# florianwechsung/alfi

Measured on AMD Instinct MI355X. Metric: V-cycles/sec on ldc3d P2-P0 (DoF*smooths/sec in dof_smooths_per_s), higher is better.
Workload: dtype f64

## Files before the change

### alfi_amd/csrc/api_patches.hip

```cpp
#include <optional>
#include "api_internal.h"
#include "find_groups.h"

static_assert(PLAN_E_ARG == ALFI_E_ARG, "the planners (patch_plan.h) return the C ABI's code");


static void free_f32(alfi_level* L) {
  if (L->inv32 && --L->ctx->f32_levels == 0) {
    dev_free(L->ctx->f32_work);
    L->ctx->f32_work = nullptr;
    L->ctx->f32_work_doubles = 0;
  }
  dev_free(L->inv32);
  dev_free(L->inv32_ptr);
  L->inv32 = nullptr;
  L->inv32_ptr = nullptr;
  L->inv32_floats = 0;
  std::vector<int64_t>().swap(L->f32_ptr);
  if (L->held == HELD_F32) set_held(L, HELD_NONE);
}

static int inv_to_placeholder(alfi_level* L) {
  dev_free(L->inv);
  L->inv = nullptr;
// ... 512 lines not shown
  std::vector<std::vector<int32_t>> si(ng);
  for (int g = 0; g < ng; ++g) {
    mat[g].resize((size_t)cond_group_doubles(g_m[g], g_sc[g]));
    si[g].resize(g_sc[g]);
    ALFI_HIP_CHECK(ctx, down(mat[g].data(), cd.mat + g_mat[g], sizeof(double) * mat[g].size()));
    ALFI_HIP_CHECK(ctx, down(si[g].data(), cd.sidx + g_sidx[g], sizeof(int32_t) * g_sc[g]));
  }
  std::vector<double> x(n), y(n), rhs(s);
  for (int j = 0; j < n; ++j) {
    std::fill(x.begin(), x.end(), 0.0);
    x[j] = 1.0;
    for (int i = 0; i < s; ++i) rhs[i] = x[nI + i];
    for (int g = 0; g < ng; ++g) {
      const int m = g_m[g], sc = g_sc[g], o = g_off[g], ldm = cond_ldim(m), ldsc = cond_ldim(sc);
      const double* X = mat[g].data();
      const double* B = X + (size_t)ldm * m;
      for (int i = 0; i < m; ++i) {
        double acc = 0.0;
        for (int k = 0; k < m; ++k) acc += X[(size_t)k * ldm + i] * x[o + k];
        y[o + i] = acc;
      }
      for (int i = 0; i < sc; ++i) {
        double acc = 0.0;
        for (int k = 0; k < m; ++k) acc += B[(size_t)k * ldsc + i] * y[o + k];
        rhs[si[g][i]] -= acc;
      }
    }
    for (int i = 0; i < s; ++i) {
      double acc = 0.0;
      for (int k = 0; k < s; ++k) acc += sinv[patch_inv_index(i, k, s, ld)] * rhs[k];
      y[nI + i] = acc;
    }
    for (int g = 0; g < ng; ++g) {
      const int m = g_m[g], sc = g_sc[g], o = g_off[g], ldm = cond_ldim(m);
      const double* W = mat[g].data() + (size_t)ldm * m + (size_t)cond_ldim(sc) * m;
      for (int i = 0; i < m; ++i) {
        double acc = 0.0;
        for (int k = 0; k < sc; ++k) acc += W[(size_t)k * ldm + i] * y[nI + si[g][k]];
        y[o + i] -= acc;
// ... 31 lines not shown
```

### alfi_amd/csrc/cond_layout.h

```cpp
#pragma once
#include <cstdint>

#ifdef __HIPCC__
#define ALFI_HD __host__ __device__
#else
#define ALFI_HD
#endif

struct CondChunk {
  int64_t off;
  int64_t ubase;
  int64_t sidx0;
  int64_t stage_off;
  int32_t xq0, xq1;
  int32_t bq0, bq1;
  int32_t e0, ne;
  int32_t u0, nu;
  int32_t nI;
  int32_t xp0, bp0;
  int32_t pad;
};

#ifndef ALFI_COND_SIGMA_ROWS
#define ALFI_COND_SIGMA_ROWS 64
#endif
constexpr int COND_SIGMA_ROWS = ALFI_COND_SIGMA_ROWS;

constexpr int64_t COND_PER_PATCH_MIN = 1024;

ALFI_HD inline int cond_patch_waves(int max_pairs) {
#ifdef ALFI_COND_WAVES_FORCE
  (void)max_pairs;
  return ALFI_COND_WAVES_FORCE;
#else
  return max_pairs <= 64 ? 1 : max_pairs <= 128 ? 2 : max_pairs <= 256 ? 4 : 8;
#endif
}

ALFI_HD inline int cond_ldim(int rows) { return (rows + 1) & ~1; }
ALFI_HD inline int cond_pairs(int rows) { return (rows + 1) / 2; }
ALFI_HD inline int64_t cond_group_doubles(int m, int sc) {
  return (int64_t)cond_ldim(m) * m + (int64_t)cond_ldim(sc) * m + (int64_t)cond_ldim(m) * sc;
}
```

### alfi_amd/csrc/kernels_bigpatch.hip

```cpp
#include <algorithm>
#include <cstdlib>
#include <vector>
#include "common.h"
#include "row_piece.h"
#include "cond_apply.h"

constexpr int BIG_NB = 64;
constexpr int BIG_MAX_NP = PATCH_MAX;

template <int BS>
__global__ __launch_bounds__(256) void big_gather_kernel(int64_t p0, const int32_t* __restrict__ rowptr,
                                                          const int32_t* __restrict__ colidx,
                                                          const double* __restrict__ vals, int flat,
                                                          const int64_t* __restrict__ patch_ptr,
                                                          const int32_t* __restrict__ patch_dofs,
                                                          const int64_t* __restrict__ scr_ptr, double* __restrict__ scr) {
  __shared__ int32_t dofs_s[BIG_MAX_NP];
  const int64_t p = p0 + blockIdx.y;
  const int64_t off = patch_ptr[p];
  const int n = (int)(patch_ptr[p + 1] - off);
  const int N = (n + BIG_NB - 1) / BIG_NB * BIG_NB;
  double* S = scr + scr_ptr[blockIdx.y];
  for (int i = threadIdx.x; i < n; i += 256) dofs_s[i] = patch_dofs[off + i];
  const int chunk = (N + gridDim.x - 1) / gridDim.x;
// ... 749 lines not shown
    const int m = cd.g_m[g], sc = cd.g_sc[g];
    const int ldm = cond_ldim(m), ldsc = cond_ldim(sc);
    const double* B = cd.mat + cd.g_mat[g] + (int64_t)ldm * m;
    const double* W = B + (int64_t)ldsc * m;
    const int32_t* si = cd.sidx + cd.g_sidx[g];
    for (int e = threadIdx.x; e < sc * sc; e += 256) {
      const int i = e % sc, j = e / sc;
      double acc = 0.0;
      for (int k = 0; k < m; ++k) acc = __builtin_fma(B[(int64_t)k * ldsc + i], W[(int64_t)j * ldm + k], acc);
      S[(int64_t)si[i] * N + si[j]] -= acc;
    }
    __syncthreads();
  }
}



template <bool NT, int COND_WAVES, int RU>
__global__ __launch_bounds__(64 * COND_WAVES) void cond_front_kernel(int64_t p0, int64_t p1, CondDev cd,
                                                                     const int64_t* __restrict__ patch_ptr,
                                                                     const int64_t* __restrict__ stage_ptr,
                                                                     const double* __restrict__ x, double* __restrict__ stage,
                                                                     int ordered) {
  extern __shared__ double cond_dsmem[];
  constexpr int NT_ = 64 * COND_WAVES;
  if (p0 + blockIdx.x >= p1) return;
  const int64_t p = ordered ? cd.order[blockIdx.x] : p0 + blockIdx.x;
  const int64_t off = patch_ptr[p];
  const int n = (int)(patch_ptr[p + 1] - off);
  const int nI = cd.p_nI[p];
  const int s = n - nI;
  const int64_t uo0 = cd.uptr[p];
  double* xs = cond_dsmem;
  double* ts = xs + n;
  double* us = ts + nI;
  for (int i0 = threadIdx.x; i0 < n; i0 += 4 * NT_) {
    int32_t d[4];
#pragma unroll
    for (int u = 0; u < 4; ++u) d[u] = (i0 + u * NT_ < n) ? cd.dofs[off + i0 + u * NT_] : 0;
    double v[4];
#pragma unroll
    for (int u = 0; u < 4; ++u) v[u] = (i0 + u * NT_ < n) ? x[d[u]] : 0.0;
#pragma unroll
    for (int u = 0; u < 4; ++u)
      if (i0 + u * NT_ < n) xs[i0 + u * NT_] = v[u];
  }
  __syncthreads();
  double* tmp = cd.tmp + off;
  const int64_t xp0 = cd.xp_ptr[p], bp0 = cd.bp_ptr[p];
  const int nxp = (int)(cd.xp_ptr[p + 1] - xp0), nbp = (int)(cd.bp_ptr[p + 1] - bp0);
  for (int q0 = 0; q0 < nxp; q0 += NT_) {
    const int q = q0 + threadIdx.x;
    const bool act = q < nxp;
    const int32_t g = act ? cd.xp_grp[xp0 + q] : (int32_t)cd.gptr[p];
    const int m = cd.g_m[g], o = cd.g_off[g], i = 2 * (q - cd.g_xp[g]);
    double t0 = 0.0, t1 = 0.0;
    cond_row2_dot<NT, RU>(cd.mat + cd.g_mat[g] + i, cond_ldim(m), act ? m : 0, xs + o, t0, t1);
    if (act) {
      ts[o + i] = t0;
      tmp[o + i] = t0;
      if (i + 1 < m) {
        ts[o + i + 1] = t1;
        tmp[o + i + 1] = t1;
      }
    }
  }
  __syncthreads();
  for (int q0 = 0; q0 < nbp; q0 += NT_) {
    const int q = q0 + threadIdx.x;
    const bool act = q < nbp;
    const int32_t g = act ? cd.bp_grp[bp0 + q] : (int32_t)cd.gptr[p];
    const int m = cd.g_m[g], sc = cd.g_sc[g], j = 2 * (q - cd.g_bp[g]);
    const int64_t ue = uo0 + cd.g_uoff[g] + j;
    const int32_t d0 = act ? cd.u_dst[ue] : 0, d1 = (act && j + 1 < sc) ? cd.u_dst[ue + 1] : 0;
    double u0 = 0.0, u1 = 0.0;
    cond_row2_dot<NT, RU>(cd.mat + cd.g_mat[g] + (int64_t)cond_ldim(m) * m + j, cond_ldim(sc), act ? m : 0,
                          ts + cd.g_off[g], u0, u1);
    if (act) {
      us[d0] = u0;
      if (j + 1 < sc) us[d1] = u1;
    }
  }
  __syncthreads();
  const int64_t srow0 = cd.sptr[p];
  const int32_t qb = cd.s_uptr[srow0];
  double* rhs = stage + stage_ptr[p] + nI;
  for (int i = threadIdx.x; i < s; i += NT_) {
    double acc = xs[nI + i];
    const int32_t qe = cd.s_uptr[srow0 + i + 1] - qb;
    for (int32_t q = cd.s_uptr[srow0 + i] - qb; q < qe; ++q) acc -= us[q];
    rhs[i] = acc;
  }
}

template <bool NT>
// ... 19 lines not shown
  const int lg = __builtin_ctz(R) - 1;
  const bool ahead = a < b && s <= BIG_U * (64 >> lg);
  big_d2 sv[BIG_U];
  if (ahead) big_block_prefetch<NT>(cd.sinv + cd.sinv_ptr[p] + (int64_t)row0 * s + (a - row0), P, s, lg, lane, sv);
  for (int i = threadIdx.x; i < s; i += 256) cond_dsmem[i] = rhs[i];
  __syncthreads();
  double* ys = cd.tmp + off + nI;
  if (ahead) {
    big_block_finish(sv, s, lg, cond_dsmem, lane, ys + a, s - a);
    if (a + R < b) big_rows<NT>(cd.sinv + cd.sinv_ptr[p], s, ld, a + R, b, cond_dsmem, lane, ys);
  } else if (a < b) {
    big_rows<NT>(cd.sinv + cd.sinv_ptr[p], s, ld, a, b, cond_dsmem, lane, ys);
  }
}

template <bool NT, int COND_WAVES, int RU>
__global__ __launch_bounds__(64 * COND_WAVES) void cond_back_kernel(int64_t p0, int64_t p1, CondDev cd,
                                                                    const int64_t* __restrict__ patch_ptr,
                                                                    const int64_t* __restrict__ stage_ptr,
                                                                    double* __restrict__ stage, int ordered) {
  extern __shared__ double cond_dsmem[];
  constexpr int NT_ = 64 * COND_WAVES;
  if (p0 + blockIdx.x >= p1) return;
  const int64_t p = ordered ? cd.order[blockIdx.x] : p0 + blockIdx.x;
  const int64_t off = patch_ptr[p];
  const int n = (int)(patch_ptr[p + 1] - off);
  const int nI = cd.p_nI[p];
  const int s = n - nI;
  const int uo = (int)(cd.uptr[p + 1] - cd.uptr[p]);
  const int64_t g0 = cd.gptr[p];
  double* ys = cond_dsmem;
  double* yg = ys + s;
  const double* tmp = cd.tmp + off;
  for (int i = threadIdx.x; i < s; i += NT_) ys[i] = tmp[nI + i];
  const int32_t* si = cd.sidx + (uo > 0 ? cd.g_sidx[g0] : 0);
  int32_t sq[4];
#pragma unroll
  for (int u = 0; u < 4; ++u) sq[u] = (threadIdx.x + u * NT_ < uo) ? si[threadIdx.x + u * NT_] : 0;
  __syncthreads();
#pragma unroll
  for (int u = 0; u < 4; ++u)
    if (threadIdx.x + u * NT_ < uo) yg[threadIdx.x + u * NT_] = ys[sq[u]];
  for (int q = threadIdx.x + 4 * NT_; q < uo; q += NT_) yg[q] = ys[si[q]];
  __syncthreads();
  double* out = stage + stage_ptr[p];
  const int64_t xp0 = cd.xp_ptr[p];
  const int nxp = (int)(cd.xp_ptr[p + 1] - xp0);
  for (int q0 = 0; q0 < nxp; q0 += NT_) {
// ... 66 lines not shown
  d.boff = cd.g_mat[g] + (int64_t)cond_ldim(m) * m + j;
  d.ld = cond_ldim(sc);
  d.m = m;
  d.o = cd.g_off[g];
  d.d0 = cd.u_dst[ue];
  d.d1 = j + 1 < sc ? cd.u_dst[ue + 1] : -1;
  d.pad = 0;
  return d;
}

template <bool NT>
__global__ __launch_bounds__(256) void cond_gfront_kernel(int64_t k0, CondDev cd, const double* __restrict__ x) {
  extern __shared__ double cond_dsmem[];
  const CondChunk c = cd.gc[k0 + blockIdx.x];
  double* xs = cond_dsmem;
  double* ts = xs + c.ne;
  const int tid = threadIdx.x;
  const bool xact = c.xq0 + tid < c.xq1, bact = c.bq0 + tid < c.bq1;
  const CondXPair xd = cond_xpair(cd, c, c.xq0 + tid, xact);
  const CondBPair bd = cond_bpair(cd, c, c.bq0 + tid, bact);
  for (int i = tid; i < c.ne; i += 256) xs[i] = x[cd.dofs[c.off + c.e0 + i]];
  big_d2 xa[COND_U], ba[COND_U];
  cond_row2_prefetch<NT>(cd.mat + xd.xoff, xd.ld, xact ? xd.m : 0, xa);
  cond_row2_prefetch<NT>(cd.mat + bd.boff, bd.ld, bact ? bd.m : 0, ba);
  __syncthreads();
  double* tmp = cd.tmp + c.off;
  {
    double t0 = 0.0, t1 = 0.0;
    cond_row2_finish<NT>(cd.mat + xd.xoff, xd.ld, xact ? xd.m : 0, xs + (xd.o - c.e0), xa, t0, t1);
    if (xact) {
      const int e = xd.o + xd.i;
      ts[e - c.e0] = t0;
      tmp[e] = t0;
      if (xd.sl1 >= 0) {
        ts[e - c.e0 + 1] = t1;
        tmp[e + 1] = t1;
      }
    }
  }
  __syncthreads();
  {
    double v0 = 0.0, v1 = 0.0;
    cond_row2_finish<NT>(cd.mat + bd.boff, bd.ld, bact ? bd.m : 0, ts + (bd.o - c.e0), ba, v0, v1);
    if (bact) {
      cd.ubuf[c.ubase + bd.d0] = v0;
      if (bd.d1 >= 0) cd.ubuf[c.ubase + bd.d1] = v1;
    }
  }
}

template <bool NT>
__global__ __launch_bounds__(256) void cond_gsigma_kernel(int64_t c0, CondDev cd, const int64_t* __restrict__ patch_ptr,
                                                          const int64_t* __restrict__ stage_ptr, const double* __restrict__ x,
                                                          double* __restrict__ stage) {
  extern __shared__ double cond_dsmem[];
  const int64_t c = c0 + blockIdx.x;
  const int64_t p = cd.ch_patch[c];
  const int r0 = cd.ch_row[c];
// ... 106 lines not shown
        hipLaunchKernelGGL(cond_fill_kernel<3>, dim3((unsigned)nb), block, lds, ctx->stream, p0, K->cd, K->patch_ptr,
                           K->patch_dofs, K->A.rowptr, K->A.colidx, K->A.vals, K->A.flat, d_scr_ptr, dst, K->status);
      const int64_t ga = K->cplan.gptr[p0], gb = K->cplan.gptr[p0 + nb];
      if (gb > ga && pivot_groups) {
        const size_t glds = (size_t)(COND_GMAX * COND_GMAX + 64 * COND_GMAX) * sizeof(double) + COND_GMAX * sizeof(int);
        (void)hipFuncSetAttribute(reinterpret_cast<const void*>(&cond_group_pivot_kernel),
                                  hipFuncAttributeMaxDynamicSharedMemorySize, (int)glds);
        hipLaunchKernelGGL(cond_group_pivot_kernel, dim3((unsigned)(gb - ga)), dim3(64), glds, ctx->stream, ga, K->cd, K->status);
      } else if (gb > ga && K->cplan.max_m <= 16)
        hipLaunchKernelGGL(cond_group16_kernel, dim3((unsigned)((gb - ga + 15) / 16)), block, 0, ctx->stream, ga, gb, K->cd,
                           K->status);
      else if (gb > ga)
        hipLaunchKernelGGL(cond_group_kernel, dim3((unsigned)((gb - ga + 3) / 4)), block, 0, ctx->stream, ga, gb, K->cd,
                           K->status);
      hipLaunchKernelGGL(cond_schur_kernel, dim3((unsigned)nb), block, 0, ctx->stream, p0, K->cd, K->patch_ptr, d_scr_ptr, dst);
    } else if (C) {
      const int64_t n = C->n, N = (n + BIG_NB - 1) / BIG_NB * BIG_NB;
      hipLaunchKernelGGL(coarse_pad_kernel, dim3(8192), block, 0, ctx->stream, n, N, dst);
      if (C->bs == 2)
        hipLaunchKernelGGL(coarse_scatter_kernel<2>, dim3(4096), block, 0, ctx->stream, C->A.nbrows, C->A.rowptr, C->A.colidx,
                           C->A.vals, C->A.flat, N, dst);
      else
        hipLaunchKernelGGL(coarse_scatter_kernel<3>, dim3(4096), block, 0, ctx->stream, C->A.nbrows, C->A.rowptr, C->A.colidx,
                           C->A.vals, C->A.flat, N, dst);
    } else if (T) {
      hipLaunchKernelGGL(big_dense_fill_kernel, dim3(64, (unsigned)nb), block, 0, ctx->stream, p0, T->m, T->KII, T->DII,
                         T->nu, T->gamma, d_scr_ptr, dst);
    } else {
      if (L->bs == 2)
        hipLaunchKernelGGL(big_gather_kernel<2>, dim3(16, (unsigned)nb), block, 0, ctx->stream, p0, L->A.rowptr, L->A.colidx,
// ... 206 lines not shown
    const int64_t k0 = L->cplan.gcptr[p0], k1 = L->cplan.gcptr[p1];
    const size_t lds_f = (size_t)L->cplan.lds_gfront, lds_b = (size_t)L->cplan.lds_gback;
    const size_t lds_s = (size_t)(L->cplan.max_s + 2 + COND_SIGMA_ROWS) * sizeof(double);
    if (k1 > k0)
      hipLaunchKernelGGL((cond_gfront_kernel<false>), dim3((unsigned)(k1 - k0)), dim3(256), lds_f, ctx->stream, k0, L->cd, x);
    if (c1 > c0)
      hipLaunchKernelGGL((cond_gsigma_kernel<true>), dim3((unsigned)(c1 - c0)), dim3(256), lds_s, ctx->stream, c0, L->cd,
                         L->patch_ptr, L->stage_ptr, x, L->stage);
    if (k1 > k0)
      hipLaunchKernelGGL((cond_gback_kernel<false>), dim3((unsigned)(k1 - k0)), dim3(256), lds_b, ctx->stream, k0, L->cd,
                         L->stage);
    ALFI_HIP_CHECK(ctx, hipGetLastError());
    return 0;
  }
  const size_t lds_f = (size_t)L->cplan.lds_front, lds_s = (size_t)(L->cplan.max_s + 2) * sizeof(double);
  const size_t lds_b = (size_t)L->cplan.lds_back;
#define ALFI_COND_LAUNCH3(WV)                                                                                             \
  do {                                                                                                                    \
    if (lds_f > 64 * 1024)                                                                                                \
      ALFI_HIP_CHECK(ctx, hipFuncSetAttribute(reinterpret_cast<const void*>(&cond_front_kernel<false, WV, 8>),            \
                                              hipFuncAttributeMaxDynamicSharedMemorySize, (int)lds_f));                   \
    hipLaunchKernelGGL((cond_front_kernel<false, WV, 8>), dim3(grid.x), dim3(64 * WV), lds_f, ctx->stream, p0, p1, L->cd, \
                       L->patch_ptr, L->stage_ptr, x, L->stage, ordered);                                                 \
    if (c1 > c0)                                                                                                          \
      hipLaunchKernelGGL((cond_sigma_kernel<true>), dim3((unsigned)(c1 - c0)), dim3(256), lds_s, ctx->stream, c0, L->cd,  \
                         L->patch_ptr, L->stage_ptr, L->stage);                                                           \
    if (lds_b > 64 * 1024)                                                                                                \
      ALFI_HIP_CHECK(ctx, hipFuncSetAttribute(reinterpret_cast<const void*>(&cond_back_kernel<false, WV, 8>),             \
                                              hipFuncAttributeMaxDynamicSharedMemorySize, (int)lds_b));                   \
    hipLaunchKernelGGL((cond_back_kernel<false, WV, 8>), dim3(grid.x), dim3(64 * WV), lds_b, ctx->stream, p0, p1, L->cd,  \
                       L->patch_ptr, L->stage_ptr, L->stage, ordered);                                                    \
  } while (0)
#ifdef ALFI_COND_WAVES_FORCE
  ALFI_COND_LAUNCH3(ALFI_COND_WAVES_FORCE);
#else
  switch (cond_patch_waves(L->cplan.max_pairs)) {
    case 1: ALFI_COND_LAUNCH3(1); break;
    case 2: ALFI_COND_LAUNCH3(2); break;
    case 4: ALFI_COND_LAUNCH3(4); break;
    default: ALFI_COND_LAUNCH3(8); break;
  }
#endif
#undef ALFI_COND_LAUNCH3
  ALFI_HIP_CHECK(ctx, hipGetLastError());
  return 0;
}

#include "mf_coarse.h"
```

### alfi_amd/csrc/kernels_block_cond.hip

```cpp
#include "common.h"
#include "row_piece.h"
#include "block_cols.h"
#include "cond_apply.h"

template <bool NT, int COND_WAVES, int RU, int NV>
__global__ __launch_bounds__(64 * COND_WAVES) void cond_front_block_kernel(int64_t p0, int64_t p1, CondDev cd,
                                                                           const int64_t* __restrict__ patch_ptr,
                                                                           const int64_t* __restrict__ stage_ptr,
                                                                           const double* __restrict__ X, int64_t ldx, BlockCols cols,
                                                                           double* __restrict__ stage, int64_t stage_len,
                                                                           double* __restrict__ ctmp, int64_t ctmp_len, int ordered) {
  extern __shared__ double cond_dsmem[];
  constexpr int NT_ = 64 * COND_WAVES;
  if (p0 + blockIdx.x >= p1) return;
  const int64_t p = ordered ? cd.order[blockIdx.x] : p0 + blockIdx.x;
  const int64_t off = patch_ptr[p];
  const int n = (int)(patch_ptr[p + 1] - off);
  const int nI = cd.p_nI[p];
  const int s = n - nI;
  const int64_t uo0 = cd.uptr[p];
  double* xs = cond_dsmem;
  double* ts = xs + n * NV;
  double* us = ts + nI * NV;
  for (int i0 = threadIdx.x; i0 < n; i0 += 4 * NT_) {
    int32_t d[4];
#pragma unroll
    for (int u = 0; u < 4; ++u) d[u] = (i0 + u * NT_ < n) ? cd.dofs[off + i0 + u * NT_] : 0;
    double v[4][NV];
#pragma unroll
    for (int u = 0; u < 4; ++u)
#pragma unroll
      for (int c = 0; c < NV; ++c) v[u][c] = (i0 + u * NT_ < n) ? X[(int64_t)cols.c[c] * ldx + d[u]] : 0.0;
#pragma unroll
    for (int u = 0; u < 4; ++u)
      if (i0 + u * NT_ < n) {
#pragma unroll
        for (int c = 0; c < NV; ++c) xs[(i0 + u * NT_) * NV + c] = v[u][c];
      }
// ... 2 lines not shown
  double* tmp = ctmp + off;
  const int64_t xp0 = cd.xp_ptr[p], bp0 = cd.bp_ptr[p];
  const int nxp = (int)(cd.xp_ptr[p + 1] - xp0), nbp = (int)(cd.bp_ptr[p + 1] - bp0);
  for (int q0 = 0; q0 < nxp; q0 += NT_) {
    const int q = q0 + threadIdx.x;
    const bool act = q < nxp;
    const int32_t g = act ? cd.xp_grp[xp0 + q] : (int32_t)cd.gptr[p];
    const int m = cd.g_m[g], o = cd.g_off[g], i = 2 * (q - cd.g_xp[g]);
    double t[NV][2];
#pragma unroll
    for (int c = 0; c < NV; ++c) t[c][0] = t[c][1] = 0.0;
    cond_row2_dot<NT, RU, NV>(cd.mat + cd.g_mat[g] + i, cond_ldim(m), act ? m : 0, xs + o * NV, t);
    if (act) {
#pragma unroll
      for (int c = 0; c < NV; ++c) {
        ts[(o + i) * NV + c] = t[c][0];
        tmp[c * ctmp_len + o + i] = t[c][0];
        if (i + 1 < m) {
          ts[(o + i + 1) * NV + c] = t[c][1];
          tmp[c * ctmp_len + o + i + 1] = t[c][1];
        }
      }
    }
  }
  __syncthreads();
  for (int q0 = 0; q0 < nbp; q0 += NT_) {
    const int q = q0 + threadIdx.x;
    const bool act = q < nbp;
    const int32_t g = act ? cd.bp_grp[bp0 + q] : (int32_t)cd.gptr[p];
    const int m = cd.g_m[g], sc = cd.g_sc[g], j = 2 * (q - cd.g_bp[g]);
    const int64_t ue = uo0 + cd.g_uoff[g] + j;
    const int32_t d0 = act ? cd.u_dst[ue] : 0, d1 = (act && j + 1 < sc) ? cd.u_dst[ue + 1] : 0;
    double u[NV][2];
#pragma unroll
    for (int c = 0; c < NV; ++c) u[c][0] = u[c][1] = 0.0;
    cond_row2_dot<NT, RU, NV>(cd.mat + cd.g_mat[g] + (int64_t)cond_ldim(m) * m + j, cond_ldim(sc), act ? m : 0,
                              ts + cd.g_off[g] * NV, u);
    if (act) {
#pragma unroll
      for (int c = 0; c < NV; ++c) {
        us[d0 * NV + c] = u[c][0];
        if (j + 1 < sc) us[d1 * NV + c] = u[c][1];
      }
    }
  }
  __syncthreads();
  const int64_t srow0 = cd.sptr[p];
  const int32_t qb = cd.s_uptr[srow0];
  double* rhs = stage + stage_ptr[p] + nI;
  for (int i = threadIdx.x; i < s; i += NT_) {
    double acc[NV];
#pragma unroll
// ... 181 lines not shown
```

### alfi_amd/csrc/patch_plan.h

```cpp
#pragma once
#include <algorithm>
#include <climits>
#include <cstdarg>
#include <cstdint>
#include <cstdio>
#include <string>
#include <vector>
#include "cond_layout.h"

#pragma GCC visibility push(hidden)

constexpr int PLAN_E_ARG = -2;
constexpr int SMALL_PATCH_MAX = 160;
constexpr int PATCH_MAX = 4096;
constexpr int COND_LDS_MAX_BYTES = 150 * 1024;
constexpr int COND_GROUP_MAX = 64;
constexpr int COND_CHUNK_PAIRS = 256;
constexpr int MULT_WAVE_NODES = 64;

inline int plan_fail(std::string* err, const char* fmt, ...) {
  char buf[1024];
  va_list ap;
  va_start(ap, fmt);
  vsnprintf(buf, sizeof(buf), fmt, ap);
// ... 132 lines not shown
}

struct CondPlan {
  std::vector<int32_t> dofs, slot;
  std::vector<int64_t> gptr, g_mat, g_sidx;
  std::vector<int32_t> g_off, g_m, g_sc, g_uoff, g_xp, g_bp;
  std::vector<int32_t> sidx;
  std::vector<int32_t> p_nI, order;
  std::vector<int64_t> sptr, sinv_ptr, uptr, xp_ptr, bp_ptr;
  std::vector<int32_t> s_uptr, s_uidx, u_dst;
  std::vector<int64_t> chptr, gcptr;
  std::vector<int32_t> ch_patch, ch_row, xp_grp, bp_grp;
  std::vector<CondChunk> gc;
  int64_t ngroups = 0, mat_doubles = 0, sinv_doubles = 0;
  int lds_bytes = 0, lds_front = 0, lds_back = 0, lds_gfront = 0, lds_gback = 0;
  int max_s = 0;
  int max_m = 0;
  int max_pairs = 0;
  int umax = 0;

  void release_tables() {
    CondPlan keep;
    keep.sptr.swap(sptr); keep.gptr.swap(gptr); keep.chptr.swap(chptr); keep.gcptr.swap(gcptr);
    keep.ngroups = ngroups; keep.mat_doubles = mat_doubles; keep.sinv_doubles = sinv_doubles;
    keep.lds_bytes = lds_bytes; keep.lds_front = lds_front; keep.lds_back = lds_back;
    keep.lds_gfront = lds_gfront; keep.lds_gback = lds_gback;
    keep.max_s = max_s; keep.max_m = max_m; keep.max_pairs = max_pairs; keep.umax = umax;
    *this = std::move(keep);
  }
};

inline int plan_condensed(int bs, int64_t nb, int64_t npatch, const int64_t* pp, const int32_t* pd, const int32_t* group,
                          const int32_t* rowptr, const int32_t* colidx, int sigma_rows, CondPlan* out, std::string* err) {
  const int64_t sum_n = pp[npatch];
  std::vector<int32_t> c_dofs(sum_n), c_slot(sum_n), g_off, g_m, g_sc, g_uoff, sidx, p_nI(npatch), s_uptr, s_uidx;
  std::vector<int64_t> gptr(npatch + 1, 0), g_mat, g_sidx, sptr(npatch + 1, 0), sinv_ptr(npatch + 1, 0);
  std::vector<int32_t> node_pos(nb, -1);
  int64_t mat_off = 0, sinv_off = 0;
  int lds_max = 0, umax = 0, smax = 0;
  s_uptr.push_back(0);
  for (int64_t p = 0; p < npatch; ++p) {
// ... 93 lines not shown
  if (s_uidx.empty()) s_uidx.push_back(0);
  std::vector<int32_t> order((size_t)npatch);
  {
    std::vector<int64_t> pbytes((size_t)npatch, 0);
    for (int64_t p = 0; p < npatch; ++p) {
      const int64_t s = sptr[p + 1] - sptr[p];
      pbytes[p] = s * s;
      for (int64_t g = gptr[p]; g < gptr[p + 1]; ++g) pbytes[p] += cond_group_doubles(g_m[g], g_sc[g]);
    }
    for (int64_t p = 0; p < npatch; ++p) order[p] = (int32_t)p;
    std::stable_sort(order.begin(), order.end(), [&](int32_t a, int32_t b) { return pbytes[a] > pbytes[b]; });
  }
  std::vector<int32_t> ch_patch, ch_row, xp_grp, bp_grp, g_xp(g_m.size()), g_bp(g_m.size()), u_dst;
  std::vector<int64_t> chptr((size_t)npatch + 1, 0), uptr((size_t)npatch + 1, 0), xp_ptr((size_t)npatch + 1, 0),
      bp_ptr((size_t)npatch + 1, 0);
  int lds_front = 0, lds_back = 0, max_pairs = 0;
  for (int64_t p = 0; p < npatch; ++p) {
    const int s = (int)(sptr[p + 1] - sptr[p]), ld = (s + 1) & ~1;
    for (int r = 0; r < ld; r += sigma_rows) {
      ch_patch.push_back((int32_t)p);
      ch_row.push_back(r);
    }
    chptr[p + 1] = (int64_t)ch_patch.size();
    int uo = 0, xp = 0, bp = 0;
    for (int64_t g = gptr[p]; g < gptr[p + 1]; ++g) {
      g_xp[g] = xp;
      g_bp[g] = bp;
      for (int i = 0; i < cond_pairs(g_m[g]); ++i) xp_grp.push_back((int32_t)g);
      for (int j = 0; j < cond_pairs(g_sc[g]); ++j) bp_grp.push_back((int32_t)g);
      xp += cond_pairs(g_m[g]);
      bp += cond_pairs(g_sc[g]);
      uo += g_sc[g];
    }
    uptr[p + 1] = uptr[p] + uo;
    xp_ptr[p + 1] = xp_ptr[p] + xp;
    bp_ptr[p + 1] = bp_ptr[p] + bp;
    const int32_t qb = s_uptr[sptr[p]], qe = s_uptr[sptr[p + 1]];
    if (qe - qb != uo) return plan_fail(err, "patch %lld: inconsistent skeleton contributions", (long long)p);
    u_dst.resize((size_t)uptr[p + 1]);
    for (int32_t q = qb; q < qe; ++q) u_dst[uptr[p] + s_uidx[q]] = q - qb;
    max_pairs = std::max(max_pairs, std::max(xp, bp));
    lds_front = std::max(lds_front, (int)((pp[p + 1] - pp[p] + p_nI[p] + uo + 2) * (int64_t)sizeof(double)));
    lds_back = std::max(lds_back, (int)((s + uo + 2) * (int64_t)sizeof(double)));
  }
  if (ch_patch.empty()) { ch_patch.push_back(0); ch_row.push_back(0); }
  if (xp_grp.empty()) xp_grp.push_back(0);
  if (bp_grp.empty()) bp_grp.push_back(0);
  if (u_dst.empty()) u_dst.push_back(0);
  if (lds_front > COND_LDS_MAX_BYTES) return plan_fail(err, "condensed apply would need %d bytes of LDS per patch", lds_front);
  std::vector<CondChunk> gc;
  std::vector<int64_t> gcptr((size_t)npatch + 1, 0), stage_off((size_t)npatch + 1, 0);
  for (int64_t p = 0; p < npatch; ++p)
    stage_off[p + 1] = stage_off[p] + ((pp[p + 1] - pp[p] + 1) & ~(int64_t)1);
  int lds_gf = 0, lds_gb = 0;
  for (int64_t p = 0; p < npatch; ++p) {
    int64_t g = gptr[p];
    while (g < gptr[p + 1]) {
      CondChunk c;
// ... 15 lines not shown
      lds_gf = std::max(lds_gf, (int)(2 * ne * sizeof(double)));
      lds_gb = std::max(lds_gb, (int)(nu * sizeof(double)));
    }
    gcptr[p + 1] = (int64_t)gc.size();
  }
  if (xp_ptr[npatch] > INT32_MAX || bp_ptr[npatch] > INT32_MAX)
    return plan_fail(err, "condensed factors: too many row pairs on one level");
  if (gc.empty()) gc.push_back(CondChunk());
  CondPlan& o = *out;
  o.ngroups = (int64_t)g_off.size();
  o.mat_doubles = mat_off;
  o.sinv_doubles = sinv_off;
  o.lds_bytes = lds_max;
  o.lds_front = lds_front;
  o.lds_back = lds_back;
  o.lds_gfront = lds_gf + 16;
  o.lds_gback = lds_gb + 16;
  o.max_s = smax;
  o.max_m = g_m.empty() ? 0 : *std::max_element(g_m.begin(), g_m.end());
  o.max_pairs = max_pairs;
  o.umax = umax;
  o.dofs = std::move(c_dofs); o.slot = std::move(c_slot);
  o.gptr = std::move(gptr); o.g_mat = std::move(g_mat); o.g_sidx = std::move(g_sidx);
  o.g_off = std::move(g_off); o.g_m = std::move(g_m); o.g_sc = std::move(g_sc); o.g_uoff = std::move(g_uoff);
  o.g_xp = std::move(g_xp); o.g_bp = std::move(g_bp);
  o.sidx = std::move(sidx);
  o.p_nI = std::move(p_nI); o.order = std::move(order);
  o.sptr = std::move(sptr); o.sinv_ptr = std::move(sinv_ptr); o.uptr = std::move(uptr);
  o.xp_ptr = std::move(xp_ptr); o.bp_ptr = std::move(bp_ptr);
  o.s_uptr = std::move(s_uptr); o.s_uidx = std::move(s_uidx); o.u_dst = std::move(u_dst);
// ... 123 lines not shown
```

Measured before the change: 7.936.

## Pre-multiply coupling blocks by interior inverse to shorten condensed apply chain

```diff
diff --git a/alfi_amd/csrc/api_patches.hip b/alfi_amd/csrc/api_patches.hip
--- a/alfi_amd/csrc/api_patches.hip
+++ b/alfi_amd/csrc/api_patches.hip
@@ -550,7 +550,7 @@
     for (int g = 0; g < ng; ++g) {
       const int m = g_m[g], sc = g_sc[g], o = g_off[g], ldm = cond_ldim(m), ldsc = cond_ldim(sc);
       const double* X = mat[g].data();
-      const double* B = X + (size_t)ldm * m;
+      const double* C = X + (size_t)ldm * m;
       for (int i = 0; i < m; ++i) {
         double acc = 0.0;
         for (int k = 0; k < m; ++k) acc += X[(size_t)k * ldm + i] * x[o + k];
@@ -558,7 +558,7 @@
       }
       for (int i = 0; i < sc; ++i) {
         double acc = 0.0;
-        for (int k = 0; k < m; ++k) acc += B[(size_t)k * ldsc + i] * y[o + k];
+        for (int k = 0; k < m; ++k) acc += C[(size_t)k * ldsc + i] * x[o + k];
         rhs[si[g][i]] -= acc;
       }
     }
diff --git a/alfi_amd/csrc/cond_layout.h b/alfi_amd/csrc/cond_layout.h
--- a/alfi_amd/csrc/cond_layout.h
+++ b/alfi_amd/csrc/cond_layout.h
@@ -37,6 +37,16 @@
 #endif
 }
 
+ALFI_HD inline bool cond_star_schedule(int max_pairs) {
+#ifdef ALFI_COND_STAR_FORCE
+  return ALFI_COND_STAR_FORCE != 0 && max_pairs <= 128;
+#else
+  return max_pairs <= 128;
+#endif
+}
+
+ALFI_HD inline int64_t cond_back_star_doubles(int64_t s, int64_t uo, int64_t nI) { return s + uo + 3 * nI + 2; }
+
 ALFI_HD inline int cond_ldim(int rows) { return (rows + 1) & ~1; }
 ALFI_HD inline int cond_pairs(int rows) { return (rows + 1) / 2; }
 ALFI_HD inline int64_t cond_group_doubles(int m, int sc) {
diff --git a/alfi_amd/csrc/kernels_bigpatch.hip b/alfi_amd/csrc/kernels_bigpatch.hip
--- a/alfi_amd/csrc/kernels_bigpatch.hip
+++ b/alfi_amd/csrc/kernels_bigpatch.hip
@@ -787,9 +787,88 @@
   }
 }
 
-
-
-template <bool NT, int COND_WAVES, int RU>
+template <int GM>
+__device__ __forceinline__ void cond_bx_body(int m, int sc, int ldm, int ldsc, const double* __restrict__ X, double* __restrict__ B,
+                                           int lane) {
+  constexpr int KU = GM > 24 ? 2 : 4;
+  double acc[GM];
+#pragma unroll
+  for (int j = 0; j < GM; ++j) acc[j] = 0.0;
+  for (int k0 = 0; k0 < m; k0 += KU) {
+    double bk[KU], xk[KU];
+#pragma unroll
+    for (int u = 0; u < KU; ++u) {
+      bk[u] = (lane < sc && k0 + u < m) ? B[(int64_t)(k0 + u) * ldsc + lane] : 0.0;
+      xk[u] = (lane < m && k0 + u < m) ? X[(int64_t)lane * ldm + k0 + u] : 0.0;
+    }
+#pragma unroll
+    for (int u = 0; u < KU; ++u) {
+#pragma unroll
+      for (int j = 0; j < GM; ++j) acc[j] = __builtin_fma(bk[u], __shfl(xk[u], j, 64), acc[j]);
+    }
+  }
+#pragma unroll
+  for (int j = 0; j < GM; ++j)
+    if (lane < sc && j < m) B[(int64_t)j * ldsc + lane] = acc[j];
+}
+
+template <int GMAX>
+__global__ __launch_bounds__(256) void cond_bx_kernel(int64_t g_begin, int64_t g_end, CondDev cd) {
+  const int64_t g = g_begin + (int64_t)blockIdx.x * 4 + (threadIdx.x >> 6);
+  if (g >= g_end) return;
+  const int lane = threadIdx.x & 63;
+  const int m = cd.g_m[g], sc = cd.g_sc[g];
+  const int ldm = cond_ldim(m), ldsc = cond_ldim(sc);
+  const double* X = cd.mat + cd.g_mat[g];
+  double* B = cd.mat + cd.g_mat[g] + (int64_t)ldm * m;
+  if (m <= 4) cond_bx_body<4>(m, sc, ldm, ldsc, X, B, lane);
+  else if (m <= 12) cond_bx_body<12>(m, sc, ldm, ldsc, X, B, lane);
+  else if (m <= 16) cond_bx_body<16>(m, sc, ldm, ldsc, X, B, lane);
+  else if constexpr (GMAX > 16) {
+    if (m <= 24) cond_bx_body<24>(m, sc, ldm, ldsc, X, B, lane);
+    else if (m <= 46) cond_bx_body<46>(m, sc, ldm, ldsc, X, B, lane);
+    else cond_bx_body<COND_GMAX>(m, sc, ldm, ldsc, X, B, lane);
+  }
+}
+
+
+
+template <int NT_>
+__device__ __forceinline__ void cond_gather(const int32_t* __restrict__ dofs, int n, const double* __restrict__ x,
+                                            double* __restrict__ xs) {
+  for (int i0 = threadIdx.x; i0 < n; i0 += 4 * NT_) {
+    int32_t d[4];
+#pragma unroll
+    for (int u = 0; u < 4; ++u) d[u] = (i0 + u * NT_ < n) ? dofs[i0 + u * NT_] : 0;
+    double v[4];
+#pragma unroll
+    for (int u = 0; u < 4; ++u) v[u] = (i0 + u * NT_ < n) ? x[d[u]] : 0.0;
+#pragma unroll
+    for (int u = 0; u < 4; ++u)
+      if (i0 + u * NT_ < n) xs[i0 + u * NT_] = v[u];
+  }
+}
+
+struct CondCPair {
+  const double* M;
+  int ld, kn, o, d0, d1;
+};
+__device__ __forceinline__ CondCPair cond_cpair(const CondDev& cd, int64_t bp0, int64_t uo0, int q, bool act) {
+  CondCPair c = {cd.mat, 2, 0, 0, 0, -1};
+  if (!act) return c;
+  const int32_t g = cd.bp_grp[bp0 + q];
+  const int m = cd.g_m[g], sc = cd.g_sc[g], j = 2 * (q - cd.g_bp[g]);
+  const int64_t ue = uo0 + cd.g_uoff[g] + j;
+  c.M = cd.mat + cd.g_mat[g] + (int64_t)cond_ldim(m) * m + j;
+  c.ld = cond_ldim(sc);
+  c.kn = m;
+  c.o = cd.g_off[g];
+  c.d0 = cd.u_dst[ue];
+  c.d1 = j + 1 < sc ? cd.u_dst[ue + 1] : -1;
+  return c;
+}
+
+template <bool NT, int COND_WAVES, int RU, bool STAR>
 __global__ __launch_bounds__(64 * COND_WAVES) void cond_front_kernel(int64_t p0, int64_t p1, CondDev cd,
                                                                      const int64_t* __restrict__ patch_ptr,
                                                                      const int64_t* __restrict__ stage_ptr,
@@ -803,55 +882,63 @@
   const int n = (int)(patch_ptr[p + 1] - off);
   const int nI = cd.p_nI[p];
   const int s = n - nI;
-  const int64_t uo0 = cd.uptr[p];
+  const int64_t uo0 = cd.uptr[p], g0 = cd.gptr[p];
+  const int64_t bp0 = cd.bp_ptr[p];
+  const int nbp = (int)(cd.bp_ptr[p + 1] - bp0);
   double* xs = cond_dsmem;
-  double* ts = xs + n;
-  double* us = ts + nI;
-  for (int i0 = threadIdx.x; i0 < n; i0 += 4 * NT_) {
-    int32_t d[4];
-#pragma unroll
-    for (int u = 0; u < 4; ++u) d[u] = (i0 + u * NT_ < n) ? cd.dofs[off + i0 + u * NT_] : 0;
-    double v[4];
-#pragma unroll
-    for (int u = 0; u < 4; ++u) v[u] = (i0 + u * NT_ < n) ? x[d[u]] : 0.0;
-#pragma unroll
-    for (int u = 0; u < 4; ++u)
-      if (i0 + u * NT_ < n) xs[i0 + u * NT_] = v[u];
-  }
-  __syncthreads();
-  double* tmp = cd.tmp + off;
-  const int64_t xp0 = cd.xp_ptr[p], bp0 = cd.bp_ptr[p];
-  const int nxp = (int)(cd.xp_ptr[p + 1] - xp0), nbp = (int)(cd.bp_ptr[p + 1] - bp0);
-  for (int q0 = 0; q0 < nxp; q0 += NT_) {
-    const int q = q0 + threadIdx.x;
-    const bool act = q < nxp;
-    const int32_t g = act ? cd.xp_grp[xp0 + q] : (int32_t)cd.gptr[p];
-    const int m = cd.g_m[g], o = cd.g_off[g], i = 2 * (q - cd.g_xp[g]);
-    double t0 = 0.0, t1 = 0.0;
-    cond_row2_dot<NT, RU>(cd.mat + cd.g_mat[g] + i, cond_ldim(m), act ? m : 0, xs + o, t0, t1);
-    if (act) {
-      ts[o + i] = t0;
-      tmp[o + i] = t0;
-      if (i + 1 < m) {
-        ts[o + i + 1] = t1;
-        tmp[o + i + 1] = t1;
-      }
-    }
-  }
-  __syncthreads();
-  for (int q0 = 0; q0 < nbp; q0 += NT_) {
-    const int q = q0 + threadIdx.x;
-    const bool act = q < nbp;
-    const int32_t g = act ? cd.bp_grp[bp0 + q] : (int32_t)cd.gptr[p];
-    const int m = cd.g_m[g], sc = cd.g_sc[g], j = 2 * (q - cd.g_bp[g]);
-    const int64_t ue = uo0 + cd.g_uoff[g] + j;
-    const int32_t d0 = act ? cd.u_dst[ue] : 0, d1 = (act && j + 1 < sc) ? cd.u_dst[ue + 1] : 0;
-    double u0 = 0.0, u1 = 0.0;
-    cond_row2_dot<NT, RU>(cd.mat + cd.g_mat[g] + (int64_t)cond_ldim(m) * m + j, cond_ldim(sc), act ? m : 0,
-                          ts + cd.g_off[g], u0, u1);
-    if (act) {
-      us[d0] = u0;
-      if (j + 1 < sc) us[d1] = u1;
+  double* us = xs + n;
+  if constexpr (STAR) {
+    const bool act0 = (int)threadIdx.x < nbp;
+    const CondCPair c0 = cond_cpair(cd, bp0, uo0, threadIdx.x, act0);
+    cond_gather<NT_>(cd.dofs + off, n, x, xs);
+    __syncthreads();
+    {
+      double u0 = 0.0, u1 = 0.0;
+      cond_row2_dot<NT, RU>(c0.M, c0.ld, c0.kn, xs + c0.o, u0, u1);
+      if (act0) {
+        us[c0.d0] = u0;
+        if (c0.d1 >= 0) us[c0.d1] = u1;
+      }
+    }
+    for (int q0 = NT_; q0 < nbp; q0 += NT_) {
+      const int q = q0 + threadIdx.x;
+      const bool act = q < nbp;
+      const CondCPair c = cond_cpair(cd, bp0, uo0, q, act);
+      double u0 = 0.0, u1 = 0.0;
+      cond_row2_dot<NT, RU>(c.M, c.ld, c.kn, xs + c.o, u0, u1);
+      if (act) {
+        us[c.d0] = u0;
+        if (c.d1 >= 0) us[c.d1] = u1;
+      }
+    }
+  } else {
+    cond_gather<NT_>(cd.dofs + off, n, x, xs);
+    __syncthreads();
+    double* tmp = cd.tmp + off;
+    const int64_t xp0 = cd.xp_ptr[p];
+    const int nxp = (int)(cd.xp_ptr[p + 1] - xp0);
+    for (int q0 = 0; q0 < nxp; q0 += NT_) {
+      const int q = q0 + threadIdx.x;
+      const bool act = q < nxp;
+      const int32_t g = act ? cd.xp_grp[xp0 + q] : (int32_t)g0;
+      const int m = cd.g_m[g], o = cd.g_off[g], i = 2 * (q - cd.g_xp[g]);
+      double t0 = 0.0, t1 = 0.0;
+      cond_row2_dot<NT, RU>(cd.mat + cd.g_mat[g] + i, cond_ldim(m), act ? m : 0, xs + o, t0, t1);
+      if (act) {
+        tmp[o + i] = t0;
+        if (i + 1 < m) tmp[o + i + 1] = t1;
+      }
+    }
+    for (int q0 = 0; q0 < nbp; q0 += NT_) {
+      const int q = q0 + threadIdx.x;
+      const bool act = q < nbp;
+      const CondCPair c = cond_cpair(cd, bp0, uo0, q, act);
+      double u0 = 0.0, u1 = 0.0;
+      cond_row2_dot<NT, RU>(c.M, c.ld, c.kn, xs + c.o, u0, u1);
+      if (act) {
+        us[c.d0] = u0;
+        if (c.d1 >= 0) us[c.d1] = u1;
+      }
     }
   }
   __syncthreads();
@@ -901,11 +988,37 @@
   }
 }
 
-template <bool NT, int COND_WAVES, int RU>
+struct CondBackItem {
+  const double* M;
+  const double* v;
+  int ld, kn, dst;
+  bool two;
+};
+__device__ __forceinline__ CondBackItem cond_back_item(const CondDev& cd, int64_t xp0, int nxp, int nI, int k, bool act,
+                                                       const double* xI, const double* yg) {
+  CondBackItem it = {cd.mat, xI, 2, 0, 0, false};
+  if (!act) return it;
+  const bool isw = k < nxp;
+  const int q = isw ? k : k - nxp;
+  const int32_t g = cd.xp_grp[xp0 + q];
+  const int m = cd.g_m[g], sc = cd.g_sc[g], o = cd.g_off[g], i = 2 * (q - cd.g_xp[g]);
+  const int ldm = cond_ldim(m);
+  const double* X = cd.mat + cd.g_mat[g] + i;
+  it.M = isw ? X + (int64_t)ldm * m + (int64_t)cond_ldim(sc) * m : X;
+  it.v = isw ? yg + cd.g_uoff[g] : xI + o;
+  it.ld = ldm;
+  it.kn = isw ? sc : m;
+  it.dst = (isw ? nI : 0) + o + i;
+  it.two = i + 1 < m;
+  return it;
+}
+
+template <bool NT, int COND_WAVES, int RU, bool STAR>
 __global__ __launch_bounds__(64 * COND_WAVES) void cond_back_kernel(int64_t p0, int64_t p1, CondDev cd,
                                                                     const int64_t* __restrict__ patch_ptr,
                                                                     const int64_t* __restrict__ stage_ptr,
-                                                                    double* __restrict__ stage, int ordered) {
+                                                                    const double* __restrict__ x, double* __restrict__ stage,
+                                                                    int ordered) {
   extern __shared__ double cond_dsmem[];
   constexpr int NT_ = 64 * COND_WAVES;
   if (p0 + blockIdx.x >= p1) return;
@@ -919,6 +1032,58 @@
   double* ys = cond_dsmem;
   double* yg = ys + s;
   const double* tmp = cd.tmp + off;
+  if constexpr (STAR) {
+    double* xI = yg + uo;
+    double* tw = xI + nI;
+    double* out = stage + stage_ptr[p];
+    const int64_t xp0 = cd.xp_ptr[p];
+    const int nxp = (int)(cd.xp_ptr[p + 1] - xp0);
+    const int tid = threadIdx.x;
+    const bool act0 = tid < 2 * nxp;
+    const CondBackItem it0 = cond_back_item(cd, xp0, nxp, nI, tid, act0, xI, yg);
+    const int32_t* si = cd.sidx + (uo > 0 ? cd.g_sidx[g0] : 0);
+    int32_t sq[4], slI[2];
+#pragma unroll
+    for (int u = 0; u < 4; ++u) sq[u] = (tid + u * NT_ < uo) ? si[tid + u * NT_] : 0;
+#pragma unroll
+    for (int u = 0; u < 2; ++u) slI[u] = (tid + u * NT_ < nI) ? cd.slot[off + tid + u * NT_] : 0;
+    const int32_t slS = tid < s ? cd.slot[off + nI + tid] : 0;
+    for (int i = tid; i < s; i += NT_) ys[i] = tmp[nI + i];
+    cond_gather<NT_>(cd.dofs + off, nI, x, xI);
+    __syncthreads();
+#pragma unroll
+    for (int u = 0; u < 4; ++u)
+      if (tid + u * NT_ < uo) yg[tid + u * NT_] = ys[sq[u]];
+    for (int q = tid + 4 * NT_; q < uo; q += NT_) yg[q] = ys[si[q]];
+    __syncthreads();
+    {
+      double a0 = 0.0, a1 = 0.0;
+      cond_row2_dot<NT, RU>(it0.M, it0.ld, it0.kn, it0.v, a0, a1);
+      if (act0) {
+        tw[it0.dst] = a0;
+        if (it0.two) tw[it0.dst + 1] = a1;
+      }
+    }
+    for (int k0 = NT_; k0 < 2 * nxp; k0 += NT_) {
+      const int k = k0 + tid;
+      const bool act = k < 2 * nxp;
+      const CondBackItem it = cond_back_item(cd, xp0, nxp, nI, k, act, xI, yg);
+      double a0 = 0.0, a1 = 0.0;
+      cond_row2_dot<NT, RU>(it.M, it.ld, it.kn, it.v, a0, a1);
+      if (act) {
+        tw[it.dst] = a0;
+        if (it.two) tw[it.dst + 1] = a1;
+      }
+    }
+    __syncthreads();
+#pragma unroll
+    for (int u = 0; u < 2; ++u)
+      if (tid + u * NT_ < nI) out[slI[u]] = tw[tid + u * NT_] - tw[nI + tid + u * NT_];
+    for (int e = tid + 2 * NT_; e < nI; e += NT_) out[cd.slot[off + e]] = tw[e] - tw[nI + e];
+    if (tid < s) out[slS] = ys[tid];
+    for (int i = tid + NT_; i < s; i += NT_) out[cd.slot[off + nI + i]] = ys[i];
+    return;
+  }
   for (int i = threadIdx.x; i < s; i += NT_) ys[i] = tmp[nI + i];
   const int32_t* si = cd.sidx + (uo > 0 ? cd.g_sidx[g0] : 0);
   int32_t sq[4];
@@ -1015,7 +1180,6 @@
   extern __shared__ double cond_dsmem[];
   const CondChunk c = cd.gc[k0 + blockIdx.x];
   double* xs = cond_dsmem;
-  double* ts = xs + c.ne;
   const int tid = threadIdx.x;
   const bool xact = c.xq0 + tid < c.xq1, bact = c.bq0 + tid < c.bq1;
   const CondXPair xd = cond_xpair(cd, c, c.xq0 + tid, xact);
@@ -1031,18 +1195,13 @@
     cond_row2_finish<NT>(cd.mat + xd.xoff, xd.ld, xact ? xd.m : 0, xs + (xd.o - c.e0), xa, t0, t1);
     if (xact) {
       const int e = xd.o + xd.i;
-      ts[e - c.e0] = t0;
       tmp[e] = t0;
-      if (xd.sl1 >= 0) {
-        ts[e - c.e0 + 1] = t1;
-        tmp[e + 1] = t1;
-      }
-    }
-  }
-  __syncthreads();
+      if (xd.sl1 >= 0) tmp[e + 1] = t1;
+    }
+  }
   {
     double v0 = 0.0, v1 = 0.0;
-    cond_row2_finish<NT>(cd.mat + bd.boff, bd.ld, bact ? bd.m : 0, ts + (bd.o - c.e0), ba, v0, v1);
+    cond_row2_finish<NT>(cd.mat + bd.boff, bd.ld, bact ? bd.m : 0, xs + (bd.o - c.e0), ba, v0, v1);
     if (bact) {
       cd.ubuf[c.ubase + bd.d0] = v0;
       if (bd.d1 >= 0) cd.ubuf[c.ubase + bd.d1] = v1;
@@ -1179,6 +1338,10 @@
         hipLaunchKernelGGL(cond_group_kernel, dim3((unsigned)((gb - ga + 3) / 4)), block, 0, ctx->stream, ga, gb, K->cd,
                            K->status);
       hipLaunchKernelGGL(cond_schur_kernel, dim3((unsigned)nb), block, 0, ctx->stream, p0, K->cd, K->patch_ptr, d_scr_ptr, dst);
+      if (gb > ga && K->cplan.max_m <= 16)
+        hipLaunchKernelGGL(cond_bx_kernel<16>, dim3((unsigned)((gb - ga + 3) / 4)), block, 0, ctx->stream, ga, gb, K->cd);
+      else if (gb > ga)
+        hipLaunchKernelGGL(cond_bx_kernel<COND_GMAX>, dim3((unsigned)((gb - ga + 3) / 4)), block, 0, ctx->stream, ga, gb, K->cd);
     } else if (C) {
       const int64_t n = C->n, N = (n + BIG_NB - 1) / BIG_NB * BIG_NB;
       hipLaunchKernelGGL(coarse_pad_kernel, dim3(8192), block, 0, ctx->stream, n, N, dst);
@@ -1415,31 +1578,34 @@
     return 0;
   }
   const size_t lds_f = (size_t)L->cplan.lds_front, lds_s = (size_t)(L->cplan.max_s + 2) * sizeof(double);
-  const size_t lds_b = (size_t)L->cplan.lds_back;
-#define ALFI_COND_LAUNCH3(WV)                                                                                             \
-  do {                                                                                                                    \
-    if (lds_f > 64 * 1024)                                                                                                \
-      ALFI_HIP_CHECK(ctx, hipFuncSetAttribute(reinterpret_cast<const void*>(&cond_front_kernel<false, WV, 8>),            \
-                                              hipFuncAttributeMaxDynamicSharedMemorySize, (int)lds_f));                   \
-    hipLaunchKernelGGL((cond_front_kernel<false, WV, 8>), dim3(grid.x), dim3(64 * WV), lds_f, ctx->stream, p0, p1, L->cd, \
-                       L->patch_ptr, L->stage_ptr, x, L->stage, ordered);                                                 \
-    if (c1 > c0)                                                                                                          \
-      hipLaunchKernelGGL((cond_sigma_kernel<true>), dim3((unsigned)(c1 - c0)), dim3(256), lds_s, ctx->stream, c0, L->cd,  \
-                         L->patch_ptr, L->stage_ptr, L->stage);                                                           \
-    if (lds_b > 64 * 1024)                                                                                                \
-      ALFI_HIP_CHECK(ctx, hipFuncSetAttribute(reinterpret_cast<const void*>(&cond_back_kernel<false, WV, 8>),             \
-                                              hipFuncAttributeMaxDynamicSharedMemorySize, (int)lds_b));                   \
-    hipLaunchKernelGGL((cond_back_kernel<false, WV, 8>), dim3(grid.x), dim3(64 * WV), lds_b, ctx->stream, p0, p1, L->cd,  \
-                       L->patch_ptr, L->stage_ptr, L->stage, ordered);                                                    \
+  const int waves = cond_patch_waves(L->cplan.max_pairs);
+  const bool star = waves <= 2 && cond_star_schedule(L->cplan.max_pairs);
+  const size_t lds_b = (size_t)(star ? L->cplan.lds_back_star : L->cplan.lds_back);
+#define ALFI_COND_LAUNCH3(WV, STAR)                                                                                        \
+  do {                                                                                                                     \
+    if (lds_f > 64 * 1024)                                                                                                 \
+      ALFI_HIP_CHECK(ctx, hipFuncSetAttribute(reinterpret_cast<const void*>(&cond_front_kernel<false, WV, 8, STAR>),       \
+                                              hipFuncAttributeMaxDynamicSharedMemorySize, (int)lds_f));                    \
+    hipLaunchKernelGGL((cond_front_kernel<false, WV, 8, STAR>), dim3(grid.x), dim3(64 * WV), lds_f, ctx->stream, p0, p1,   \
+                       L->cd, L->patch_ptr, L->stage_ptr, x, L->stage, ordered);                                           \
+    if (c1 > c0)                                                                                                           \
+      hipLaunchKernelGGL((cond_sigma_kernel<true>), dim3((unsigned)(c1 - c0)), dim3(256), lds_s, ctx->stream, c0, L->cd,   \
+                         L->patch_ptr, L->stage_ptr, L->stage);                                                            \
+    if (lds_b > 64 * 1024)                                                                                                 \
+      ALFI_HIP_CHECK(ctx, hipFuncSetAttribute(reinterpret_cast<const void*>(&cond_back_kernel<false, WV, 8, STAR>),        \
+                                              hipFuncAttributeMaxDynamicSharedMemorySize, (int)lds_b));                    \
+    hipLaunchKernelGGL((cond_back_kernel<false, WV, 8, STAR>), dim3(grid.x), dim3(64 * WV), lds_b, ctx->stream, p0, p1,    \
+                       L->cd, L->patch_ptr, L->stage_ptr, x, L->stage, ordered);                                           \
   } while (0)
 #ifdef ALFI_COND_WAVES_FORCE
-  ALFI_COND_LAUNCH3(ALFI_COND_WAVES_FORCE);
+  if (star) ALFI_COND_LAUNCH3(ALFI_COND_WAVES_FORCE, true);
+  else ALFI_COND_LAUNCH3(ALFI_COND_WAVES_FORCE, false);
 #else
-  switch (cond_patch_waves(L->cplan.max_pairs)) {
-    case 1: ALFI_COND_LAUNCH3(1); break;
-    case 2: ALFI_COND_LAUNCH3(2); break;
-    case 4: ALFI_COND_LAUNCH3(4); break;
-    default: ALFI_COND_LAUNCH3(8); break;
+  switch (waves) {
+    case 1: if (star) ALFI_COND_LAUNCH3(1, true); else ALFI_COND_LAUNCH3(1, false); break;
+    case 2: if (star) ALFI_COND_LAUNCH3(2, true); else ALFI_COND_LAUNCH3(2, false); break;
+    case 4: ALFI_COND_LAUNCH3(4, false); break;
+    default: ALFI_COND_LAUNCH3(8, false); break;
   }
 #endif
 #undef ALFI_COND_LAUNCH3
diff --git a/alfi_amd/csrc/kernels_block_cond.hip b/alfi_amd/csrc/kernels_block_cond.hip
--- a/alfi_amd/csrc/kernels_block_cond.hip
+++ b/alfi_amd/csrc/kernels_block_cond.hip
@@ -20,8 +20,7 @@
   const int s = n - nI;
   const int64_t uo0 = cd.uptr[p];
   double* xs = cond_dsmem;
-  double* ts = xs + n * NV;
-  double* us = ts + nI * NV;
+  double* us = xs + n * NV;
   for (int i0 = threadIdx.x; i0 < n; i0 += 4 * NT_) {
     int32_t d[4];
 #pragma unroll
@@ -54,16 +53,11 @@
     if (act) {
 #pragma unroll
       for (int c = 0; c < NV; ++c) {
-        ts[(o + i) * NV + c] = t[c][0];
         tmp[c * ctmp_len + o + i] = t[c][0];
-        if (i + 1 < m) {
-          ts[(o + i + 1) * NV + c] = t[c][1];
-          tmp[c * ctmp_len + o + i + 1] = t[c][1];
-        }
-      }
-    }
-  }
-  __syncthreads();
+        if (i + 1 < m) tmp[c * ctmp_len + o + i + 1] = t[c][1];
+      }
+    }
+  }
   for (int q0 = 0; q0 < nbp; q0 += NT_) {
     const int q = q0 + threadIdx.x;
     const bool act = q < nbp;
@@ -75,7 +69,7 @@
 #pragma unroll
     for (int c = 0; c < NV; ++c) u[c][0] = u[c][1] = 0.0;
     cond_row2_dot<NT, RU, NV>(cd.mat + cd.g_mat[g] + (int64_t)cond_ldim(m) * m + j, cond_ldim(sc), act ? m : 0,
-                              ts + cd.g_off[g] * NV, u);
+                              xs + cd.g_off[g] * NV, u);
     if (act) {
 #pragma unroll
       for (int c = 0; c < NV; ++c) {
diff --git a/alfi_amd/csrc/patch_plan.h b/alfi_amd/csrc/patch_plan.h
--- a/alfi_amd/csrc/patch_plan.h
+++ b/alfi_amd/csrc/patch_plan.h
@@ -170,6 +170,7 @@
   std::vector<CondChunk> gc;
   int64_t ngroups = 0, mat_doubles = 0, sinv_doubles = 0;
   int lds_bytes = 0, lds_front = 0, lds_back = 0, lds_gfront = 0, lds_gback = 0;
+  int lds_back_star = 0;
   int max_s = 0;
   int max_m = 0;
   int max_pairs = 0;
@@ -180,7 +181,7 @@
     keep.sptr.swap(sptr); keep.gptr.swap(gptr); keep.chptr.swap(chptr); keep.gcptr.swap(gcptr);
     keep.ngroups = ngroups; keep.mat_doubles = mat_doubles; keep.sinv_doubles = sinv_doubles;
     keep.lds_bytes = lds_bytes; keep.lds_front = lds_front; keep.lds_back = lds_back;
-    keep.lds_gfront = lds_gfront; keep.lds_gback = lds_gback;
+    keep.lds_gfront = lds_gfront; keep.lds_gback = lds_gback; keep.lds_back_star = lds_back_star;
     keep.max_s = max_s; keep.max_m = max_m; keep.max_pairs = max_pairs; keep.umax = umax;
     *this = std::move(keep);
   }
@@ -304,7 +305,7 @@
   std::vector<int32_t> ch_patch, ch_row, xp_grp, bp_grp, g_xp(g_m.size()), g_bp(g_m.size()), u_dst;
   std::vector<int64_t> chptr((size_t)npatch + 1, 0), uptr((size_t)npatch + 1, 0), xp_ptr((size_t)npatch + 1, 0),
       bp_ptr((size_t)npatch + 1, 0);
-  int lds_front = 0, lds_back = 0, max_pairs = 0;
+  int lds_front = 0, lds_back = 0, lds_back_star = 0, max_pairs = 0;
   for (int64_t p = 0; p < npatch; ++p) {
     const int s = (int)(sptr[p + 1] - sptr[p]), ld = (s + 1) & ~1;
     for (int r = 0; r < ld; r += sigma_rows) {
@@ -332,6 +333,7 @@
     max_pairs = std::max(max_pairs, std::max(xp, bp));
     lds_front = std::max(lds_front, (int)((pp[p + 1] - pp[p] + p_nI[p] + uo + 2) * (int64_t)sizeof(double)));
     lds_back = std::max(lds_back, (int)((s + uo + 2) * (int64_t)sizeof(double)));
+    lds_back_star = std::max(lds_back_star, (int)(cond_back_star_doubles(s, uo, p_nI[p]) * (int64_t)sizeof(double)));
   }
   if (ch_patch.empty()) { ch_patch.push_back(0); ch_row.push_back(0); }
   if (xp_grp.empty()) xp_grp.push_back(0);
@@ -377,6 +379,7 @@
   o.lds_bytes = lds_max;
   o.lds_front = lds_front;
   o.lds_back = lds_back;
+  o.lds_back_star = lds_back_star;
   o.lds_gfront = lds_gf + 16;
   o.lds_gback = lds_gb + 16;
   o.max_s = smax;
```

After: 8.003 (median of 6 runs). Within noise of the previous version (+0.8%).
